# davide-coccomini/MINTIME-Multi-Identity-size-iNvariant-TIMEsformer-for-Video-Deepfake-Detection

Measured on AMD Instinct MI355X. Metric: clips/sec (8-frame, 2-identity, 224^2 crops) fwd+bwd, higher is better.
Workload: dtype f32; 1 GPU; config 3: EfficientNet-B0 + SizeInvariantTimeSformer(dim 512, depth 9, heads 8), B=32/GPU, 8 frames, 2 identities (identity-masked), 224x224 crops, random-init seeded weights (restored before every step), train-mode BN + drop-connect 0.2, step = fwd + BCE loss + bwd + SGD(lr .01, wd 1e-4); global_batch=32, frames=8, parallelism=dp1

## Files before the change

include/mintime_hip.h:

```cpp
#ifndef MINTIME_HIP_H
#define MINTIME_HIP_H
#include <stdint.h>
#ifdef __cplusplus
extern "C" {
#endif

#define MT_VERSION 122

int mt_version(void);
const char* mt_last_error(void);

int mt_set_deterministic(int on);
int mt_get_deterministic(void);
int mt_det_release(void* stream);
int mt_det_bn_sums(const float* x, const float* z, const float* mean_invstd, int64_t rows, int C, int mode, double* stats, void* stream);

typedef struct { int gin, gout, off; } mt_rowmap;

enum { MT_OP_NT = 0,
       MT_OP_NN = 1,
       MT_OP_TN = 2 };

enum { MT_PRO_NONE = 0, MT_PRO_BN_SWISH_GATE = 1, MT_PRO_BN_SWISH = 2, MT_PRO_AFFINE = 3,
       MT_PRO_BN_BWD = 4,
// ... 53 lines not shown
  int epilogue;
  int M, N, K;
  const void* a_planes;
  const void* b_planes;
  float* C; int64_t ldc;
  const float* bias;
  const float* R; int64_t ldr;
  float* C2; int64_t ldc2;
  int n_half;
  float* col_sum;
  void* c_planes;
  int split_k;
  void* sk_workspace;
  int64_t sk_workspace_bytes;
  double* stats; int stats_slots;
} mt_gemm_planes_desc;

int mt_gemm_planes(const mt_gemm_planes_desc* d, void* stream);

int mt_mul_planes(const float* x, const float* m, void* planes, float* out, int rows, int cols, void* stream);
int mt_mul_add(const float* y, const float* m, const float* r, float* out, int64_t n, void* stream);
int mt_geglu_bwd(const float* dh, const float* m, const float* u, void* du_planes, float* du, int rows, int n_half, void* stream);
int64_t mt_gemm_planes_workspace_bytes(void);
int mt_gemm_planes_set_persist(int blocks_per_cu);


int mt_layernorm_fwd(const float* x, const float* gamma, const float* beta, float* y, float* stats,
                     int rows, int dim, float eps, void* y_planes, void* stream);

int mt_embed_fwd(float* x, const float* cls, const float* pos_emb, const float* size_emb,
                 const int64_t* positions, const int32_t* sizes, int B, int F, int n, int dim, int pos_rows, int size_rows,
// ... 232 lines not shown
```

mintime-multi-identity-size-invariant-timesformer-for-video-deepfake-detection_amd/csrc/gemm_planes.hip:

```cpp
#include "../../include/mintime_hip.h"
#include "common.hpp"
#include "gemm_planes_launch.hpp"
#include "gemm_geometry.hpp"
#include "det.hpp"
#include <string.h>

using namespace mt;

namespace {

__device__ __forceinline__ void to_blk_block(const float* __restrict__ src, int64_t ld, int R, int C, const PlaneRef& o, int rb, int cb, int lane) {
  const int r = rb * 32 + (lane >> 1), c = cb * 16 + (lane & 1) * 8;
  float x[8] = {0.f, 0.f, 0.f, 0.f, 0.f, 0.f, 0.f, 0.f};
  if (r < R) {
    const float* s = src + (int64_t)r * ld + c;
    if (c + 8 <= C && ((ld & 3) == 0) && (((uintptr_t)src & 15) == 0)) {
      const float4 u = *reinterpret_cast<const float4*>(s), v = *reinterpret_cast<const float4*>(s + 4);
      x[0] = u.x; x[1] = u.y; x[2] = u.z; x[3] = u.w; x[4] = v.x; x[5] = v.y; x[6] = v.z; x[7] = v.w;
    } else {
#pragma unroll
      for (int e = 0; e < 8; ++e) if (c + e < C) x[e] = s[e];
    }
  }
  planes_store8(o, r, c, x);
// ... 70 lines not shown
}

extern "C" int mt_gemm_planes_set_persist(int blocks_per_cu) {
  const int prev = persist_blocks();
  g_persist = blocks_per_cu < 0 || blocks_per_cu > 4 ? 0 : blocks_per_cu;
  return prev;
}

extern "C" int64_t mt_gemm_planes_workspace_bytes(void) { return kSkFlagBytes + (int64_t)kSkMaxGrid * 128 * 128 * 4; }

extern "C" int64_t mt_planes_elems(int rows, int cols) {
  if (rows <= 0 || cols <= 0) return 0;
  return (int64_t)((rows + 31) & ~31) * ((cols + 15) & ~15);
}

extern "C" int mt_split_planes_blk(const float* src, int64_t ld, int rows, int cols, void* planes, void* stream) {
  if (!src || !planes) return fail(MT_ERR_ARG, "mt_split_planes_blk: null pointer");
  if (rows <= 0 || cols <= 0 || ld < cols) return fail(MT_ERR_ARG, "mt_split_planes_blk: bad shape %d x %d (ld %lld)", rows, cols, (long long)ld);
  if ((uintptr_t)planes & 15) return fail(MT_ERR_ARG, "mt_split_planes_blk: planes must be 16-byte aligned");
  const int cb16 = (cols + 15) >> 4, rp = (rows + 31) & ~31;
  const PlaneRef o{reinterpret_cast<__bf16*>(planes), (int64_t)rp * cb16 * 16, cb16, rp};
  hipLaunchKernelGGL(split_planes_blk_kernel, dim3((cb16 + 3) / 4, rp / 32), dim3(256), 0, (hipStream_t)stream, src, ld, rows, cols, o);
  return check_launch("mt_split_planes_blk");
}

extern "C" int mt_bn_bwd_apply_planes(const float* du, const float* z, const float* kabc, void* planes, int rows, int C, void* stream) {
  if (!du || !z || !kabc || !planes || rows <= 0 || C <= 0) return fail(MT_ERR_ARG, "mt_bn_bwd_apply_planes: bad arguments");
  if ((C & 3) || (((uintptr_t)du | (uintptr_t)z | (uintptr_t)kabc | (uintptr_t)planes) & 15))
    return fail(MT_ERR_ARG, "mt_bn_bwd_apply_planes: C %% 4 == 0 and 16-byte alignment");
  const int cb16 = (C + 15) >> 4, rp = (rows + 31) & ~31;
// ... 4 lines not shown

extern "C" int mt_split_planes_blk_multi(const void* items, int count, int64_t total_blocks, void* stream) {
  if (!items || count <= 0 || total_blocks <= 0) return fail(MT_ERR_ARG, "mt_split_planes_blk_multi: bad arguments");
  hipLaunchKernelGGL(split_planes_blk_multi_kernel, dim3((unsigned)((total_blocks + 3) / 4)), dim3(256), 0, (hipStream_t)stream,
                     reinterpret_cast<const SplitItem*>(items), count, total_blocks);
  return check_launch("mt_split_planes_blk_multi");
}

static int gemm_planes_impl(const mt_gemm_planes_desc* d, void* stream) {
  if (!d || !d->a_planes || !d->b_planes) return fail(MT_ERR_ARG, "mt_gemm_planes: null operand planes");
  if (d->M <= 0 || d->N <= 0 || d->K <= 0) return fail(MT_ERR_ARG, "mt_gemm_planes: bad shape %d %d %d", d->M, d->N, d->K);
  if (((uintptr_t)d->a_planes & 15) || ((uintptr_t)d->b_planes & 15) || ((uintptr_t)d->c_planes & 15))
    return fail(MT_ERR_ARG, "mt_gemm_planes: planes must be 16-byte aligned");
  const int op = d->op, epi = d->epilogue;
  const bool cpl = d->c_planes != nullptr;
  if (!d->C && !cpl) return fail(MT_ERR_ARG, "mt_gemm_planes: no output");
  if (cpl && epi != MT_EPI_GEGLU && epi != MT_EPI_GEGLU_BWD) return fail(MT_ERR_UNSUPPORTED, "mt_gemm_planes: plane output only from the GEGLU pair");
  if (epi == MT_EPI_BIAS_RES && !d->R) return fail(MT_ERR_ARG, "mt_gemm_planes: BIAS_RES needs R");
  if (epi == MT_EPI_GEGLU && (d->n_half * 2 != d->N || (d->n_half & 63))) return fail(MT_ERR_ARG, "mt_gemm_planes GEGLU: N must be 2*n_half, n_half %% 64 == 0");
  if (epi == MT_EPI_GEGLU_BWD && (!d->C2 || d->n_half != d->N || (d->n_half & 31)))
    return fail(MT_ERR_ARG, "mt_gemm_planes GEGLU_BWD: needs C2, n_half == N and n_half %% 32 == 0");
  hipStream_t s = (hipStream_t)stream;
  const bool high = matmul_precision() == MT_PRECISION_HIGH;
  const int np = high ? 2 : 3;
  auto launch = [&](int skm, const GemmArgs& ga, dim3 g) {
    return high ? launch_planes_high(op, epi, cpl, skm, ga, g, s) : launch_planes_form<3>(op, epi, cpl, skm, ga, g, s);
  };

  const int a_rows = op == MT_OP_TN ? d->K : d->M, a_cols = op == MT_OP_TN ? d->M : d->K;
  const int b_rows = op == MT_OP_NT ? d->N : d->K, b_cols = op == MT_OP_NT ? d->K : d->N;
  GemmArgs a;
  memset(&a, 0, sizeof(a));
  a.C = d->C; a.M = d->M; a.N = d->N; a.K = d->K; a.ldc = d->ldc;
  a.a_planes = d->a_planes; a.a_pstride = mt_planes_elems(a_rows, a_cols); a.lda = (a_cols + 15) >> 4;
  a.b_planes = d->b_planes; a.b_pstride = mt_planes_elems(b_rows, b_cols); a.ldb = (b_cols + 15) >> 4;
  if (6 * a.a_pstride > 0xFFFFFFFFll || 6 * a.b_pstride > 0xFFFFFFFFll)
    return fail(MT_ERR_UNSUPPORTED, "mt_gemm_planes: an operand's planes span %lld bytes (> 4 GB: 32-bit DMA offsets); use mt_gemm for it (lib.planes_fit)",
                (long long)(6 * (a.a_pstride > a.b_pstride ? a.a_pstride : a.b_pstride)));
  a.bias = d->bias; a.R = d->R; a.ldr = d->ldr; a.C2 = d->C2; a.ldc2 = d->ldc2; a.n_half = d->n_half; a.col_sum = d->col_sum;
  a.hw = 1; a.stats_slots = d->stats_slots != 0 ? d->stats_slots : 1; a.stats = d->stats; a.b_hw = 1; a.e_hw = 1;
  if (epi == MT_EPI_STATS && !d->stats) return fail(MT_ERR_ARG, "mt_gemm_planes: STATS needs stats");
// ... 53 lines not shown
```

mintime-multi-identity-size-invariant-timesformer-for-video-deepfake-detection_amd/csrc/gemm_planes.hpp:

```cpp
#pragma once
#include "gemm_split.hpp"
#include "planes.hpp"

#ifndef MT_PLANES_ABLATE
#define MT_PLANES_ABLATE 0
#endif
#ifndef MT_PLANES_EPI_ABLATE
#define MT_PLANES_EPI_ABLATE 0
#endif
#ifndef MT_PLANES_PRIO
#define MT_PLANES_PRIO 0
#endif

namespace mt {

typedef short s16x4_t __attribute__((ext_vector_type(4)));
enum : int { BAL_NONE = 0, BAL_PAIR = 1, BAL_PHASE = 2 };

__device__ __forceinline__ void lds_dma16_s(const void* sbase, unsigned voff, unsigned lds_byte_addr) {
  unsigned keep;
  asm volatile("s_mov_b32 %0, m0\n\ts_mov_b32 m0, %3\n\ts_nop 0\n\tglobal_load_lds_dwordx4 %1, %2\n\ts_mov_b32 m0, %0"
               : "=&s"(keep) : "v"(voff), "s"(sbase), "s"(lds_byte_addr) : "memory");
}

// ... 4 lines not shown
  asm volatile("s_waitcnt lgkmcnt(0)" ::: "memory");
#pragma unroll
  for (int pass = 0; pass < 2; ++pass) {
    const int g = pass * 64 + lane, row = g >> 2, cg = g & 3;
    const float4 lo = *reinterpret_cast<const float4*>(wl + row * 36 + cg * 8);
    const float4 hi = *reinterpret_cast<const float4*>(wl + row * 36 + cg * 8 + 4);
    const int rg = row0 + row, cgl = col0 + cg * 8;
    const bool live = rg < M;
    const float x[8] = {live ? lo.x : 0.f, live ? lo.y : 0.f, live ? lo.z : 0.f, live ? lo.w : 0.f,
                        live ? hi.x : 0.f, live ? hi.y : 0.f, live ? hi.z : 0.f, live ? hi.w : 0.f};
    if (rg < o.rows_pad && cgl < o.cb16 * 16) { if (MT_PLANES_EPI_ABLATE & 8) { if (x[0] + x[7] == 123.456f) o.p[0] = (__bf16)1.f; } else planes_store8(o, rg, cgl, x); }
  }
  asm volatile("s_waitcnt lgkmcnt(0)" ::: "memory");
}

template <int TM, int TN, int EPI>
__device__ __forceinline__ void planes_epilogue(const GemmArgs& p, f32x16 (&acc)[TM][TN], int m0, int n0, int wm, int wn, int lane, float* wl) {
  static_assert(EPI == EPI_GEGLU || EPI == EPI_GEGLU_BWD, "plane output: the GEGLU pair");
  const PlaneRef o{reinterpret_cast<__bf16*>(p.c_planes), p.c_pstride, (int)p.ldcp, (p.M + 31) & ~31};
  const int col_l = lane & 31, row_h = (lane >> 5) * 4;
  const int mw = m0 + wm * TM * 32;
  if constexpr (EPI == EPI_GEGLU) {
    const int j = (n0 >> 1) + wn * 32 + col_l;
    const bool jok = j < p.n_half;
    const float ba = (jok && p.bias) ? p.bias[j] : 0.f;
    const float bg = (jok && p.bias) ? p.bias[p.n_half + j] : 0.f;
#pragma unroll
    for (int i = 0; i < TM; ++i) {
      float hv[16];
#pragma unroll
      for (int r = 0; r < 16; ++r) {
        const int m = mw + i * 32 + row_h + (r & 3) + 8 * (r >> 2);
        const float a = acc[i][0][r] + ba, g = acc[i][1][r] + bg;
        hv[r] = a * gelu_erf(g);
        if (m < p.M && jok) {
          if (p.C2) *reinterpret_cast<float2*>(p.C2 + (int64_t)m * p.ldc2 + 2 * j) = make_float2(a, g);
          if (p.C) p.C[(int64_t)m * p.ldc + j] = hv[r];
        }
      }
      planes_emit_tile(hv, wl, o, mw + i * 32, (n0 >> 1) + wn * 32, p.M, lane);
    }
  } else {
    f32x16 dgs[TM][TN];
    float s1[TN], s2[TN];
#pragma unroll
    for (int j = 0; j < TN; ++j) {
      const int n = n0 + wn * TN * 32 + j * 32 + col_l;
      const bool nok = n < p.N;
      s1[j] = 0.f; s2[j] = 0.f;
#pragma unroll
      for (int i = 0; i < TM; ++i) {
        float2 ag[16];
#pragma unroll
        for (int r = 0; r < 16; ++r) {
          const int m = mw + i * 32 + row_h + (r & 3) + 8 * (r >> 2);
          ag[r] = ((MT_PLANES_EPI_ABLATE & 1) || !(m < p.M && nok)) ? make_float2(0.3f, 0.1f)
                                                                     : *reinterpret_cast<const float2*>(p.C2 + (int64_t)m * p.ldc2 + 2 * n);
        }
#pragma unroll
        for (int r = 0; r < 16; ++r) {
          const int m = mw + i * 32 + row_h + (r & 3) + 8 * (r >> 2);
          const float v = acc[i][j][r];
          float gl, gr;
          if (MT_PLANES_EPI_ABLATE & 2) { gl = ag[r].y; gr = ag[r].y + 1.f; } else gelu_erf_both(ag[r].y, gl, gr);
          const bool live = m < p.M && nok;
          const float da = live ? v * gl : 0.f, dg = live ? v * ag[r].x * gr : 0.f;
          acc[i][j][r] = da;
          dgs[i][j][r] = dg;
          s1[j] += da; s2[j] += dg;
        }
        __builtin_amdgcn_sched_barrier(0);
      }
    }
#pragma unroll
    for (int j = 0; j < TN; ++j) {
      const int n = n0 + wn * TN * 32 + j * 32 + col_l;
      const bool nok = n < p.N;
#pragma unroll
      for (int i = 0; i < TM; ++i) {
        float da[16], dg[16];
#pragma unroll
        for (int r = 0; r < 16; ++r) {
          da[r] = acc[i][j][r]; dg[r] = dgs[i][j][r];
          const int m = mw + i * 32 + row_h + (r & 3) + 8 * (r >> 2);
          if (p.C && m < p.M && nok) { p.C[(int64_t)m * p.ldc + n] = da[r]; p.C[(int64_t)m * p.ldc + p.n_half + n] = dg[r]; }
        }
        if (MT_PLANES_EPI_ABLATE & 4) { if (da[3] + dg[5] == 123.456f) p.col_sum[0] = 1.f; }
        else if (n0 + wn * TN * 32 + j * 32 < p.N) {
          planes_emit_tile(da, wl, o, mw + i * 32, n0 + wn * TN * 32 + j * 32, p.M, lane);
          planes_emit_tile(dg, wl, o, mw + i * 32, p.n_half + n0 + wn * TN * 32 + j * 32, p.M, lane);
        }
      }
      if (p.col_sum && !(MT_PLANES_EPI_ABLATE & 16)) {
        float t1 = s1[j], t2 = s2[j];
        t1 += __shfl_xor(t1, 32);
        t2 += __shfl_xor(t2, 32);
        if (lane < 32 && nok) {
          if (p.det.vals) {
            const int rk = mw >> 5;
            det_put(p.det, n >> 5, rk, n & 31, t1);
// ... 25 lines not shown
    const int idx = t - base;
    const int per_group = rows * p.group_n;
    const int g = idx / per_group;
    const int rem = idx - g * per_group;
    const int groups = (n_tiles + p.group_n - 1) / p.group_n;
    const int gw = (g == groups - 1) ? n_tiles - g * p.group_n : p.group_n;
    const int ml = rem / gw;
    mt_ = row0 + ml;
    nt_ = g * p.group_n + (rem - ml * gw);
  } else {
    mt_ = t / n_tiles;
    nt_ = t - mt_ * n_tiles;
  }
}

template <int WAVES_M, int WAVES_N, int TM, int TN, bool AKM, bool BKM, int EPI, int STAGES, int MINW, int BAL, bool CPL = false, int SKM = 0, int NP = 3>
__global__ __launch_bounds__(WAVES_M * WAVES_N * 64, MINW)
void gemm_planes_kernel(const GemmArgs p) {
  constexpr int NW = WAVES_M * WAVES_N;
  constexpr int BM = WAVES_M * TM * 32;
  constexpr int BN = WAVES_N * TN * 32;
  constexpr int BK = 16;
  constexpr int A_PLANE = BM * 32, B_PLANE = BN * 32;
  static_assert(NP == 2 || NP == 3, "two or three pieces per operand");
  constexpr int STAGE = NP * (A_PLANE + B_PLANE);
  constexpr int PPA = A_PLANE / 1024, PPB = B_PLANE / 1024;
  constexpr int PA = NP * PPA, PB = NP * PPB;
  static_assert((PA + PB) % NW == 0, "every wavefront must issue the same number of DMA pieces");
  constexpr int IPW = (PA + PB) / NW;
  static_assert(STAGES >= 2 && STAGES <= 4, "2..4 stages");
  static_assert((!AKM || BM == 128) && (!BKM || BN == 128), "k-major images are laid out for 128-column tiles");
  constexpr bool SK = SKM == 1, PS = SKM == 2;
  static_assert(!SK || !AKM, "stream-K: forward / data-gradient forms (weight gradients split K over the grid already)");
  static_assert(!PS || (!AKM && !CPL && STAGES == 2 && EPI != EPI_GEGLU && BAL != BAL_PHASE), "persistent form: NT / NN, fp32 output, ring of two");
  constexpr bool PAIR = BAL == BAL_PAIR, PHASE = BAL == BAL_PHASE;

  extern __shared__ __attribute__((aligned(16))) unsigned char smem_pl[];
  const unsigned lds_base = (unsigned)(uintptr_t)(__attribute__((address_space(3))) unsigned char*)smem_pl;

// ... 246 lines not shown
      float sacc = 0.f;
#pragma unroll
      for (int i = 0; i < TM; ++i)
#pragma unroll
        for (int j = 0; j < TN; ++j)
#pragma unroll
          for (int r = 0; r < 16; ++r) sacc += acc[i][j][r];
      if (sacc == 123.456f) p.C[0] = sacc;
      return;
    }
    int m0e = mt_ * BM, n0e = nt_ * BN, lane_e = lane;
    asm volatile("" : "+s"(m0e), "+s"(n0e), "+v"(lane_e));
    if constexpr (CPL) {
      static_assert(!CPL || STAGES * STAGE >= NW * 32 * 36 * 4, "the plane epilogue's LDS patches live in the main loop's stages");
      __syncthreads();
      planes_epilogue<TM, TN, EPI>(p, acc, m0e, n0e, wm, wn, lane_e, reinterpret_cast<float*>(smem_pl) + wave * (32 * 36));
    } else {
      gemm_epilogue<TM, TN, EPI>(p, acc, m0e, n0e, wm, wn, lane_e, split_idx);
    }
  };

  if (p.wave_prio == 1) __builtin_amdgcn_s_setprio(1);
  else if (p.wave_prio == 2) __builtin_amdgcn_s_setprio(2);
  else if (p.wave_prio == 3) __builtin_amdgcn_s_setprio(3);
  if (MT_PLANES_PRIO == 1) {
    const unsigned hwid = __builtin_amdgcn_s_getreg((4 << 0) | (0 << 6) | (3 << 11));
    if (__builtin_amdgcn_readfirstlane(hwid) & 1) __builtin_amdgcn_s_setprio(1);
  } else if (MT_PLANES_PRIO == 2) {
    if ((blockIdx.x >> 8) & 1) __builtin_amdgcn_s_setprio(1);
  }

// ... 220 lines not shown
```

mintime-multi-identity-size-invariant-timesformer-for-video-deepfake-detection_amd/csrc/gemm_planes_high.hip:

```cpp
#include "gemm_planes_launch.hpp"

namespace mt {

int launch_planes_high(int op, int epi, bool cpl, int skm, const GemmArgs& a, dim3 grid, hipStream_t s) {
  return launch_planes_form<2>(op, epi, cpl, skm, a, grid, s);
}

}
```

mintime-multi-identity-size-invariant-timesformer-for-video-deepfake-detection_amd/csrc/gemm_planes_launch.hpp:

```cpp
#pragma once
#include "../../include/mintime_hip.h"
#include "common.hpp"
#include "gemm_planes.hpp"

#ifndef MT_PLANES_HIGH_STAGES
#define MT_PLANES_HIGH_STAGES 3
#endif

namespace mt {

template <int NP, bool AKM, bool BKM, int EPI, int BAL, bool CPL, int SK = 0>
int launch_planes(const GemmArgs& a, dim3 grid, hipStream_t s) {
  constexpr int ST = (NP == 2 && SK != 2) ? MT_PLANES_HIGH_STAGES : 2;
  auto k = gemm_planes_kernel<2, 2, 2, 2, AKM, BKM, EPI, ST, BAL == BAL_PAIR ? 2 : 3, BAL, CPL, SK, NP>;
  constexpr size_t lds = (size_t)ST * NP * (128 + 128) * 32;
  {
    hipError_t e = ensure_dynamic_lds(reinterpret_cast<const void*>(k), lds);
    if (e != hipSuccess) return fail(MT_ERR_LAUNCH, "mt_gemm_planes: cannot reserve %zu B of LDS: %s", lds, hipGetErrorString(e));
  }
  hipLaunchKernelGGL(k, grid, dim3(256), lds, s, a);
  return check_launch("mt_gemm_planes");
}

template <int NP>
int launch_planes_form(int op, int epi, bool cpl, int skm, const GemmArgs& a, dim3 grid, hipStream_t s) {
  if (op == MT_OP_TN && epi == MT_EPI_ATOMIC) return launch_planes<NP, true, true, EPI_ATOMIC, BAL_NONE, false, 0>(a, grid, s);
  if (skm == 2 && !cpl) {
    if (op == MT_OP_NT && epi == MT_EPI_STORE) return launch_planes<NP, false, false, EPI_STORE, BAL_PAIR, false, 2>(a, grid, s);
    if (op == MT_OP_NT && epi == MT_EPI_BIAS_RES) return launch_planes<NP, false, false, EPI_BIAS_RES, BAL_PAIR, false, 2>(a, grid, s);
    if (op == MT_OP_NN && epi == MT_EPI_STORE) return launch_planes<NP, false, true, EPI_STORE, BAL_PAIR, false, 2>(a, grid, s);
  }
  if (skm == 0 || skm == 1) {
#define PL_COMBO(OP, BKM_, EPI_, CPL_)                                                               \
  if (op == OP && epi == EPI_ && cpl == CPL_)                                                        \
    return skm ? launch_planes<NP, false, BKM_, EPI_, BAL_PAIR, CPL_, 1>(a, grid, s)                 \
               : launch_planes<NP, false, BKM_, EPI_, BAL_PAIR, CPL_, 0>(a, grid, s);
    PL_COMBO(MT_OP_NT, false, EPI_STORE, false)
    PL_COMBO(MT_OP_NT, false, EPI_BIAS_RES, false)
    PL_COMBO(MT_OP_NT, false, EPI_STATS, false)
    PL_COMBO(MT_OP_NT, false, EPI_GEGLU, false)
    PL_COMBO(MT_OP_NT, false, EPI_GEGLU, true)
    PL_COMBO(MT_OP_NN, true, EPI_STORE, false)
    PL_COMBO(MT_OP_NN, true, EPI_BIAS_RES, false)
    PL_COMBO(MT_OP_NN, true, EPI_GEGLU_BWD, false)
    PL_COMBO(MT_OP_NN, true, EPI_GEGLU_BWD, true)
#undef PL_COMBO
  }
  return fail(MT_ERR_UNSUPPORTED, "mt_gemm_planes: unsupported op / epilogue %d / %d", op, epi);
}

int launch_planes_high(int op, int epi, bool cpl, int skm, const GemmArgs& a, dim3 grid, hipStream_t s);

}
```

mintime-multi-identity-size-invariant-timesformer-for-video-deepfake-detection_amd/lib.py:

```python
import ctypes as C
import os
import subprocess
import threading

import torch

_HERE = os.path.dirname(os.path.abspath(__file__))
CSRC = os.path.join(_HERE, "csrc")
LIB_PATH = os.environ.get("MT_LIB") or os.path.join(CSRC, "libmintime_hip.so")

_lib = None

f32p = C.c_void_p
i64 = C.c_int64


class RowMap(C.Structure):
    _fields_ = [("gin", C.c_int), ("gout", C.c_int), ("off", C.c_int)]


class Conv3dDesc(C.Structure):
    _fields_ = [(n, C.c_int) for n in ("N", "T", "H", "W", "C", "To", "Ho", "Wo", "K", "kt", "kh", "kw", "st", "sh", "sw", "pt", "ph",
                                       "pw")] + [("ldx", i64), ("ldy", i64)]

# ... 10 lines not shown
                ("n_half", C.c_int), ("split_k", C.c_int),
                ("A2", C.c_void_p), ("b_prologue", C.c_int), ("b_scale", C.c_void_p), ("b_shift", C.c_void_p),
                ("b_gate", C.c_void_p), ("b_hw", C.c_int),
                ("conv_H", C.c_int), ("conv_W", C.c_int), ("conv_C", C.c_int), ("conv_Ho", C.c_int), ("conv_Wo", C.c_int),
                ("conv_k", C.c_int), ("conv_stride", C.c_int), ("conv_pad", C.c_int), ("conv_act", C.c_int), ("conv_src_u8", C.c_int),
                ("col_sum", C.c_void_p), ("b_planes", C.c_void_p), ("b_plane_stride", C.c_int64),
                ("e_scale", C.c_void_p), ("e_shift", C.c_void_p), ("e_gate", C.c_void_p), ("e_dpool", C.c_void_p),
                ("e_mi", C.c_void_p), ("e_hw", C.c_int)]


class GemmPlanesDesc(C.Structure):
    _fields_ = [("op", C.c_int), ("epilogue", C.c_int), ("M", C.c_int), ("N", C.c_int), ("K", C.c_int),
                ("a_planes", C.c_void_p), ("b_planes", C.c_void_p), ("C", C.c_void_p), ("ldc", i64),
                ("bias", C.c_void_p), ("R", C.c_void_p), ("ldr", i64), ("C2", C.c_void_p), ("ldc2", i64),
                ("n_half", C.c_int), ("col_sum", C.c_void_p), ("c_planes", C.c_void_p), ("split_k", C.c_int),
                ("sk_workspace", C.c_void_p), ("sk_workspace_bytes", i64), ("stats", C.c_void_p), ("stats_slots", C.c_int)]


OP_NT, OP_NN, OP_TN = 0, 1, 2
PRO_NONE, PRO_BN_SWISH_GATE, PRO_BN_SWISH, PRO_AFFINE, PRO_BN_BWD, PRO_IM2COL = 0, 1, 2, 3, 4, 5
BPRO_NONE, BPRO_BN_SWISH_GATE, BPRO_IM2COL = 0, 1, 2
EPI_STORE, EPI_BIAS_RES, EPI_GEGLU, EPI_STATS, EPI_ATOMIC, EPI_GEGLU_BWD, EPI_ACCUM, EPI_SE_RED, EPI_ACT_BWD = 0, 1, 2, 3, 4, 5, 6, 7, 8

PROTOTYPES = {
    "mt_version": [],
    "mt_last_error": [],
    "mt_set_deterministic": [C.c_int],
    "mt_get_deterministic": [],
    "mt_det_release": [C.c_void_p],
    "mt_det_bn_sums": [f32p, f32p, f32p, i64, C.c_int, C.c_int, C.c_void_p, C.c_void_p],
    "mt_gemm": [C.POINTER(GemmDesc), C.c_void_p],
    "mt_gemm_set_split": [C.c_int],
    "mt_gemm_get_split": [],
    "mt_gemm_set_precision": [C.c_int],
    "mt_gemm_get_precision": [],
    "mt_split_planes": [f32p, C.c_void_p, C.c_int64, C.c_void_p],
    "mt_planes_elems": [C.c_int, C.c_int],
    "mt_split_planes_blk": [f32p, i64, C.c_int, C.c_int, C.c_void_p, C.c_void_p],
    "mt_split_planes_blk_multi": [C.c_void_p, C.c_int, i64, C.c_void_p],
    "mt_bn_bwd_apply_planes": [f32p, f32p, f32p, C.c_void_p, C.c_int, C.c_int, C.c_void_p],
    "mt_gemm_planes": [C.POINTER(GemmPlanesDesc), C.c_void_p],
    "mt_gemm_planes_workspace_bytes": [],
    "mt_gemm_planes_set_persist": [C.c_int],
    "mt_mul_planes": [f32p, f32p, C.c_void_p, f32p, C.c_int, C.c_int, C.c_void_p],
    "mt_mul_add": [f32p, f32p, f32p, f32p, i64, C.c_void_p],
    "mt_geglu_bwd": [f32p, f32p, f32p, C.c_void_p, f32p, C.c_int, C.c_int, C.c_void_p],
    "mt_layernorm_fwd": [f32p, f32p, f32p, f32p, f32p, C.c_int, C.c_int, C.c_float, C.c_void_p, C.c_void_p],
    "mt_embed_fwd": [f32p, f32p, f32p, f32p, C.c_void_p, C.c_void_p, C.c_int, C.c_int, C.c_int, C.c_int, C.c_int, C.c_int, C.c_void_p,
                     C.c_void_p],
    "mt_attn_fwd": [f32p, f32p, f32p, C.c_void_p, C.c_void_p, C.c_int, C.c_int, C.c_int, C.c_int, C.c_int, C.c_float,
                    C.c_void_p, C.c_void_p],
    "mt_head_fwd": [f32p, f32p, f32p, f32p, f32p, f32p, C.c_int, C.c_int, C.c_int, C.c_int, C.c_float, C.c_void_p],
# ... 95 lines not shown
    "mt_sf_ingest_resize_bwd": [f32p, f32p, C.c_void_p, C.c_void_p] + [C.c_int] * 6 + [C.c_void_p, C.c_void_p, f32p] * 2 + [C.c_int] * 7 +
                               [f32p, i64, i64, i64, i64, i64, C.c_void_p],
    "mt_sf_stem_dgrad": [f32p, i64, f32p, f32p] + [C.c_int] * 6 + [C.c_void_p],
    "mt_plan_create": [C.POINTER(C.c_void_p)],
    "mt_plan_destroy": [C.c_void_p],
    "mt_plan_record_begin": [C.c_void_p],
    "mt_plan_record_end": [C.c_void_p],
    "mt_plan_size": [C.c_void_p],
    "mt_plan_tag": [C.c_int, C.c_double],
    "mt_plan_fork": [C.c_void_p, C.c_void_p],
    "mt_plan_run": [C.c_void_p, C.c_uint],
    "mt_plan_probe_read": [C.c_void_p, C.c_int, C.POINTER(C.c_int), C.POINTER(C.c_double), C.POINTER(C.c_double)],
    "mt_memset_async": [C.c_void_p, C.c_int, i64, C.c_void_p],
    "mt_copy_async": [C.c_void_p, C.c_void_p, i64, C.c_void_p],
}
_RESTYPES = {"mt_last_error": C.c_char_p, "mt_planes_elems": C.c_int64, "mt_gemm_planes_workspace_bytes": C.c_int64,
             "mt_conv3d_part_floats": C.c_int64, "mt_sf_bn_bwd_part_floats": C.c_int64}


class MintimeHipError(RuntimeError):
    pass


def build(verbose: bool = False):
    cmd = ["make", "-C", CSRC, "-j", str(min(16, os.cpu_count() or 4))]
    res = subprocess.run(cmd, capture_output=True, text=True)
    if res.returncode != 0:
        raise MintimeHipError("building libmintime_hip.so failed:\n" + res.stdout[-4000:] + res.stderr[-8000:])
    if verbose:
        print(res.stdout[-2000:])
    global _lib
# ... 125 lines not shown
    if ws is None:
        if torch.cuda.is_current_stream_capturing():
            return None
        n = get().mt_gemm_planes_workspace_bytes()
        ws = torch.zeros(n, dtype=torch.uint8, device=st.device)
        _SK_WORKSPACES[key] = ws
    return ws


def planes_fit(rows: int, cols: int) -> bool:
    rp, cp = (rows + 31) // 32 * 32, (cols + 15) // 16 * 16
    return 6 * rp * cp <= 0xFFFFFFFF


def gemm_planes(op, a_planes, b_planes, M, N, K, Cout=None, ldc=0, epilogue=EPI_STORE, bias=None, R=None, ldr=0, C2=None, ldc2=0,
                n_half=0, col_sum=None, c_planes=None, split_k=0, streamk=None, stats=None, stats_slots=0):
    d = GemmPlanesDesc()
    if streamk is None:
        streamk = os.environ.get("MT_PLANES_STREAMK", "0") != "0"
    if streamk and op != OP_TN:
        ws = streamk_workspace(a_planes.device)
        if ws is not None:
            d.sk_workspace, d.sk_workspace_bytes = ptr(ws), ws.numel()
    d.op, d.epilogue, d.M, d.N, d.K = op, epilogue, M, N, K
    d.a_planes, d.b_planes, d.C, d.ldc = ptr(a_planes), ptr(b_planes), ptr(Cout), ldc
    d.bias, d.R, d.ldr, d.C2, d.ldc2 = ptr(bias), ptr(R), ldr, ptr(C2), ldc2
    d.n_half, d.col_sum, d.c_planes, d.split_k = n_half, ptr(col_sum), ptr(c_planes), split_k
    d.stats, d.stats_slots = ptr(stats), stats_slots
    if recording() is not None:
        if op == OP_TN:
            tag_next(TAG_WGRAD, 2.0 * M * N * K)
        elif epilogue == EPI_GEGLU:
            tag_next(TAG_FF1, 2.0 * M * N * K)
    prof = PROFILE
    if prof is not None:
        for pr in prof:
            if "match_planes" in pr and pr["match_planes"](d):
                e0, e1 = torch.cuda.Event(enable_timing=True), torch.cuda.Event(enable_timing=True)
                e0.record()
                check(get().mt_gemm_planes(C.byref(d), stream_ptr()), "mt_gemm_planes")
                e1.record()
                pr["events"].append((e0, e1, 2.0 * M * N * K))
                return
# ... 282 lines not shown
```

mintime-multi-identity-size-invariant-timesformer-for-video-deepfake-detection_amd/tsf_planes.py:

```python
import os

import torch

from . import arch
from . import lib as L
from . import plans
from .lib import _new

_SEL = (2, 3, 7, 8, 12, 14)


def eligible(model, M, save):
    if os.environ.get("MT_TSF_PLANES", "1") == "0" or not L.gemm_split_enabled():
        return False
    if os.environ.get("MT_TSF_PRUNE_LAST", "0") != "0":
        return False
    if torch.cuda.is_current_stream_capturing() and save:
        return False
    D, inner = model.dim, model.heads * model.dim_head
    return (M >= 512 or dropout_active(model)) and D % 16 == 0 and inner % 16 == 0 and model.dim_head == 64


def dropout_active(model):
    return model.training and (float(model.attn_dropout) > 0.0 or float(model.ff_dropout) > 0.0)
# ... 87 lines not shown
            dm = None
            if p_att > 0.0:
                dm = _dropout_mult(model, (M, D), p_att, dev)
                y0 = _new(dev, M, D)
                L.gemm_planes(L.OP_NT, o_p, wp[(li, 3 if mode == 0 else 8)], M, D, inner, Cout=y0, ldc=D, bias=b_o)
                L.check(lib.mt_mul_add(L.ptr(y0), L.ptr(dm), L.ptr(x), L.ptr(x_new), M * D, st), "mt_mul_add")
            else:
                L.gemm_planes(L.OP_NT, o_p, wp[(li, 3 if mode == 0 else 8)], M, D, inner, Cout=x_new, ldc=D, epilogue=L.EPI_BIAS_RES,
                              bias=b_o, R=x, ldr=D)
            if save:
                rec[mode] = dict(x=x, stats=stats, xn_p=xn_p, qkv=qkv, o_p=o_p, dm=dm)
            x = x_new
        g, b_, w1, b1, w2, b2 = next(it), next(it), next(it), next(it), next(it), next(it)
        if save:
            xn_p, h_p, stats = L.planes_empty(M, D, dev), L.planes_empty(M, 4 * D, dev), _new(dev, M, 2)
            u = _new(dev, M, 8 * D)
        else:
            stats, u = None, None
        L.check(lib.mt_layernorm_fwd(L.ptr(x), L.ptr(g), L.ptr(b_), None, L.ptr(stats), M, D, eps, L.ptr(xn_p), st), "mt_layernorm_fwd")
        dm = None
        if p_ff > 0.0:
            dm = _dropout_mult(model, (M, 4 * D), p_ff, dev)
            h = _new(dev, M, 4 * D)
            L.gemm_planes(L.OP_NT, xn_p, wp[(li, 12)], M, 8 * D, D, epilogue=L.EPI_GEGLU, bias=b1, C2=u, ldc2=8 * D, n_half=4 * D,
                          Cout=h, ldc=4 * D)
            L.check(lib.mt_mul_planes(L.ptr(h), L.ptr(dm), L.ptr(h_p), None, M, 4 * D, st), "mt_mul_planes")
            del h
        else:
            L.gemm_planes(L.OP_NT, xn_p, wp[(li, 12)], M, 8 * D, D, epilogue=L.EPI_GEGLU, bias=b1, C2=u, ldc2=8 * D, n_half=4 * D,
                          c_planes=h_p)
        x_new = _new(dev, B, N, D) if save else x
        L.gemm_planes(L.OP_NT, h_p, wp[(li, 14)], M, D, 4 * D, Cout=x_new, ldc=D, epilogue=L.EPI_BIAS_RES, bias=b2, R=x, ldr=D)
        if save:
            rec[2] = dict(x=x, stats=stats, xn_p=xn_p, u=u, h_p=h_p, dm=dm)
            saved["layers"].append(rec)
        x = x_new
    g, b_, w_h, b_h = next(it), next(it), next(it), next(it)
    logits = _new(dev, B, model.num_classes)
    L.check(lib.mt_head_fwd(L.ptr(x), L.ptr(g), L.ptr(b_), L.ptr(w_h), L.ptr(b_h), L.ptr(logits), B, x.shape[1], D, model.num_classes,
                            eps, st), "mt_head_fwd")
    if save:
        saved["x_final"] = x
    return logits, s_att, t_att, saved


# ... 63 lines not shown
        i0 = take(6)
        g, b_, w1, b1, w2, b2 = P[i0:i0 + 6]
        r = rec[2]
        du_p = L.planes_empty(M, 8 * D, dev)
        dxn = torch.empty(M, D, dtype=torch.float32, device=dev)
        last = li == model.depth - 1
        wgrad(dx_p, r["h_p"], grads[i0 + 4], D, 4 * D, bias_src=dx2 if last else None, bias_out=grads[i0 + 5] if last else None)
        if r.get("dm") is not None:
            dh, du_f = torch.empty(M, 4 * D, dtype=torch.float32, device=dev), torch.empty(M, 8 * D, dtype=torch.float32, device=dev)
            L.gemm_planes(L.OP_NN, dx_p, wp[(li, 14)], M, 4 * D, D, Cout=dh, ldc=4 * D)
            L.check(lib.mt_geglu_bwd(L.ptr(dh), L.ptr(r["dm"]), L.ptr(r["u"]), L.ptr(du_p), L.ptr(du_f), M, 4 * D, st), "mt_geglu_bwd")
            side.launch(lambda du_f=du_f, out=grads[i0 + 3]: L.check(lib.mt_colsum(L.ptr(du_f), 8 * D, L.RowMap(0, 0, 0), M, 8 * D,
                                                                                 L.ptr(out), L.stream_ptr()), "mt_colsum"), reads=(du_f,))
            del dh
        else:
            L.gemm_planes(L.OP_NN, dx_p, wp[(li, 14)], M, 4 * D, D, epilogue=L.EPI_GEGLU_BWD, C2=r["u"], ldc2=8 * D, n_half=4 * D,
                          col_sum=grads[i0 + 3], c_planes=du_p)
        wgrad(du_p, r["xn_p"], grads[i0 + 2], 8 * D, D)
        L.gemm_planes(L.OP_NN, du_p, wp[(li, 12)], M, D, 8 * D, Cout=dxn, ldc=D)
        dx2, dx_p = ln_bwd(dxn, r, g, dx2, i0, None if rec[1].get("dm") is not None else grads[i0 - 1], 0)
        if not keep_saved:
            r.clear()
        for mode in (1, 0):
            i0 = take(5)
            g, b_, w_qkv, w_o, b_o = P[i0:i0 + 5]
            r = rec[mode]
            dxn = torch.empty(M, D, dtype=torch.float32, device=dev)
            dy_p = dx_p
            if r.get("dm") is not None:
                dy_p = L.planes_empty(M, D, dev)
                dy_f = torch.empty(M, D, dtype=torch.float32, device=dev)
                L.check(lib.mt_mul_planes(L.ptr(dx2), L.ptr(r["dm"]), L.ptr(dy_p), L.ptr(dy_f), M, D, st), "mt_mul_planes")
# ... 41 lines not shown
```

Baseline: 726.3 clips/s.

## Store GEGLU pre-activations in MFMA-tile order for coalesced fwd/bwd epilogue access

The GEGLU forward epilogue now writes the saved pre-activations (a, g) in a 32x32 tile-blocked layout that matches the MFMA accumulator lane order, using float4 stores. The GEGLU backward epilogue reads them back with float4 loads instead of strided per-row float2 gathers. This targets the scattered memory traffic of the large M x 8D saved tensor in both passes. It adds a C2T template variant, a new workspace-size helper and API field, and a tiled buffer that is used only when feed-forward dropout is off.

```diff
diff --git a/include/mintime_hip.h b/include/mintime_hip.h
--- a/include/mintime_hip.h
+++ b/include/mintime_hip.h
@@ -91,7 +91,10 @@
   void* sk_workspace;
   int64_t sk_workspace_bytes;
   double* stats; int stats_slots;
+  int c2_tiled;
 } mt_gemm_planes_desc;
+
+int64_t mt_geglu_tiled_elems(int M, int n_half);
 
 int mt_gemm_planes(const mt_gemm_planes_desc* d, void* stream);
 
diff --git a/mintime-multi-identity-size-invariant-timesformer-for-video-deepfake-detection_amd/csrc/gemm_planes.hip b/mintime-multi-identity-size-invariant-timesformer-for-video-deepfake-detection_amd/csrc/gemm_planes.hip
--- a/mintime-multi-identity-size-invariant-timesformer-for-video-deepfake-detection_amd/csrc/gemm_planes.hip
+++ b/mintime-multi-identity-size-invariant-timesformer-for-video-deepfake-detection_amd/csrc/gemm_planes.hip
@@ -108,6 +108,11 @@
   return (int64_t)((rows + 31) & ~31) * ((cols + 15) & ~15);
 }
 
+extern "C" int64_t mt_geglu_tiled_elems(int M, int n_half) {
+  if (M <= 0 || n_half <= 0 || (n_half & 31)) return 0;
+  return (int64_t)((M + 31) & ~31) * 2 * n_half;
+}
+
 extern "C" int mt_split_planes_blk(const float* src, int64_t ld, int rows, int cols, void* planes, void* stream) {
   if (!src || !planes) return fail(MT_ERR_ARG, "mt_split_planes_blk: null pointer");
   if (rows <= 0 || cols <= 0 || ld < cols) return fail(MT_ERR_ARG, "mt_split_planes_blk: bad shape %d x %d (ld %lld)", rows, cols, (long long)ld);
@@ -142,6 +147,10 @@
     return fail(MT_ERR_ARG, "mt_gemm_planes: planes must be 16-byte aligned");
   const int op = d->op, epi = d->epilogue;
   const bool cpl = d->c_planes != nullptr;
+  const bool c2t = d->c2_tiled != 0;
+  if (c2t && (d->c2_tiled != 1 || !((op == MT_OP_NT && epi == MT_EPI_GEGLU) || (op == MT_OP_NN && epi == MT_EPI_GEGLU_BWD)) || !cpl || !d->C2 ||
+              ((uintptr_t)d->C2 & 15)))
+    return fail(MT_ERR_ARG, "mt_gemm_planes: c2_tiled = 1 needs the GEGLU (NT) / GEGLU_BWD (NN) epilogue, c_planes and a 16-byte aligned C2");
   if (!d->C && !cpl) return fail(MT_ERR_ARG, "mt_gemm_planes: no output");
   if (cpl && epi != MT_EPI_GEGLU && epi != MT_EPI_GEGLU_BWD) return fail(MT_ERR_UNSUPPORTED, "mt_gemm_planes: plane output only from the GEGLU pair");
   if (epi == MT_EPI_BIAS_RES && !d->R) return fail(MT_ERR_ARG, "mt_gemm_planes: BIAS_RES needs R");
@@ -152,7 +161,7 @@
   const bool high = matmul_precision() == MT_PRECISION_HIGH;
   const int np = high ? 2 : 3;
   auto launch = [&](int skm, const GemmArgs& ga, dim3 g) {
-    return high ? launch_planes_high(op, epi, cpl, skm, ga, g, s) : launch_planes_form<3>(op, epi, cpl, skm, ga, g, s);
+    return high ? launch_planes_high(op, epi, cpl, skm, c2t, ga, g, s) : launch_planes_form<3>(op, epi, cpl, skm, c2t, ga, g, s);
   };
 
   const int a_rows = op == MT_OP_TN ? d->K : d->M, a_cols = op == MT_OP_TN ? d->M : d->K;
diff --git a/mintime-multi-identity-size-invariant-timesformer-for-video-deepfake-detection_amd/csrc/gemm_planes.hpp b/mintime-multi-identity-size-invariant-timesformer-for-video-deepfake-detection_amd/csrc/gemm_planes.hpp
--- a/mintime-multi-identity-size-invariant-timesformer-for-video-deepfake-detection_amd/csrc/gemm_planes.hpp
+++ b/mintime-multi-identity-size-invariant-timesformer-for-video-deepfake-detection_amd/csrc/gemm_planes.hpp
@@ -42,7 +42,7 @@
   asm volatile("s_waitcnt lgkmcnt(0)" ::: "memory");
 }
 
-template <int TM, int TN, int EPI>
+template <int TM, int TN, int EPI, bool C2T>
 __device__ __forceinline__ void planes_epilogue(const GemmArgs& p, f32x16 (&acc)[TM][TN], int m0, int n0, int wm, int wn, int lane, float* wl) {
   static_assert(EPI == EPI_GEGLU || EPI == EPI_GEGLU_BWD, "plane output: the GEGLU pair");
   const PlaneRef o{reinterpret_cast<__bf16*>(p.c_planes), p.c_pstride, (int)p.ldcp, (p.M + 31) & ~31};
@@ -56,14 +56,27 @@
 #pragma unroll
     for (int i = 0; i < TM; ++i) {
       float hv[16];
+      [[maybe_unused]] float ua[16], ug[16];
 #pragma unroll
       for (int r = 0; r < 16; ++r) {
         const int m = mw + i * 32 + row_h + (r & 3) + 8 * (r >> 2);
         const float a = acc[i][0][r] + ba, g = acc[i][1][r] + bg;
         hv[r] = a * gelu_erf(g);
+        if constexpr (C2T) { ua[r] = m < p.M ? a : 0.f; ug[r] = m < p.M ? g : 0.f; }
         if (m < p.M && jok) {
-          if (p.C2) *reinterpret_cast<float2*>(p.C2 + (int64_t)m * p.ldc2 + 2 * j) = make_float2(a, g);
+          if constexpr (!C2T) { if (p.C2) *reinterpret_cast<float2*>(p.C2 + (int64_t)m * p.ldc2 + 2 * j) = make_float2(a, g); }
           if (p.C) p.C[(int64_t)m * p.ldc + j] = hv[r];
+        }
+      }
+      if constexpr (C2T) {
+        const int rb = (mw + i * 32) >> 5, jb = ((n0 >> 1) + wn * 32) >> 5;
+        if (rb * 32 < p.M && jb * 32 < p.n_half) {
+          float* ub = p.C2 + ((int64_t)rb * (p.n_half >> 5) + jb) * 2048 + lane * 4;
+#pragma unroll
+          for (int q = 0; q < 4; ++q) {
+            *reinterpret_cast<float4*>(ub + q * 256) = make_float4(ua[4 * q], ua[4 * q + 1], ua[4 * q + 2], ua[4 * q + 3]);
+            *reinterpret_cast<float4*>(ub + 1024 + q * 256) = make_float4(ug[4 * q], ug[4 * q + 1], ug[4 * q + 2], ug[4 * q + 3]);
+          }
         }
       }
       planes_emit_tile(hv, wl, o, mw + i * 32, (n0 >> 1) + wn * 32, p.M, lane);
@@ -79,11 +92,23 @@
 #pragma unroll
       for (int i = 0; i < TM; ++i) {
         float2 ag[16];
-#pragma unroll
-        for (int r = 0; r < 16; ++r) {
-          const int m = mw + i * 32 + row_h + (r & 3) + 8 * (r >> 2);
-          ag[r] = ((MT_PLANES_EPI_ABLATE & 1) || !(m < p.M && nok)) ? make_float2(0.3f, 0.1f)
-                                                                     : *reinterpret_cast<const float2*>(p.C2 + (int64_t)m * p.ldc2 + 2 * n);
+        if constexpr (C2T) {
+          const int rb = min((mw + i * 32) >> 5, ((p.M + 31) >> 5) - 1), jb = min((n0 + wn * TN * 32 + j * 32) >> 5, (p.n_half >> 5) - 1);
+          const float* ub = p.C2 + ((int64_t)rb * (p.n_half >> 5) + jb) * 2048 + lane * 4;
+#pragma unroll
+          for (int q = 0; q < 4; ++q) {
+            float4 a4 = make_float4(0.3f, 0.3f, 0.3f, 0.3f), g4 = make_float4(0.1f, 0.1f, 0.1f, 0.1f);
+            if (!(MT_PLANES_EPI_ABLATE & 1)) { a4 = *reinterpret_cast<const float4*>(ub + q * 256); g4 = *reinterpret_cast<const float4*>(ub + 1024 + q * 256); }
+            ag[4 * q] = make_float2(a4.x, g4.x); ag[4 * q + 1] = make_float2(a4.y, g4.y);
+            ag[4 * q + 2] = make_float2(a4.z, g4.z); ag[4 * q + 3] = make_float2(a4.w, g4.w);
+          }
+        } else {
+#pragma unroll
+          for (int r = 0; r < 16; ++r) {
+            const int m = mw + i * 32 + row_h + (r & 3) + 8 * (r >> 2);
+            ag[r] = ((MT_PLANES_EPI_ABLATE & 1) || !(m < p.M && nok)) ? make_float2(0.3f, 0.1f)
+                                                                       : *reinterpret_cast<const float2*>(p.C2 + (int64_t)m * p.ldc2 + 2 * n);
+          }
         }
 #pragma unroll
         for (int r = 0; r < 16; ++r) {
@@ -100,6 +125,7 @@
         __builtin_amdgcn_sched_barrier(0);
       }
     }
+    asm volatile("" ::: "memory");
 #pragma unroll
     for (int j = 0; j < TN; ++j) {
       const int n = n0 + wn * TN * 32 + j * 32 + col_l;
@@ -110,8 +136,14 @@
 #pragma unroll
         for (int r = 0; r < 16; ++r) {
           da[r] = acc[i][j][r]; dg[r] = dgs[i][j][r];
-          const int m = mw + i * 32 + row_h + (r & 3) + 8 * (r >> 2);
-          if (p.C && m < p.M && nok) { p.C[(int64_t)m * p.ldc + n] = da[r]; p.C[(int64_t)m * p.ldc + p.n_half + n] = dg[r]; }
+        }
+        if (p.C) {
+          float* cp = p.C + (int64_t)(mw + i * 32 + row_h) * p.ldc + n;
+#pragma unroll
+          for (int r = 0; r < 16; ++r) {
+            const int dr = (r & 3) + 8 * (r >> 2);
+            if (mw + i * 32 + row_h + dr < p.M && nok) { cp[(int64_t)dr * p.ldc] = da[r]; cp[(int64_t)dr * p.ldc + p.n_half] = dg[r]; }
+          }
         }
         if (MT_PLANES_EPI_ABLATE & 4) { if (da[3] + dg[5] == 123.456f) p.col_sum[0] = 1.f; }
         else if (n0 + wn * TN * 32 + j * 32 < p.N) {
@@ -167,7 +199,7 @@
   }
 }
 
-template <int WAVES_M, int WAVES_N, int TM, int TN, bool AKM, bool BKM, int EPI, int STAGES, int MINW, int BAL, bool CPL = false, int SKM = 0, int NP = 3>
+template <int WAVES_M, int WAVES_N, int TM, int TN, bool AKM, bool BKM, int EPI, int STAGES, int MINW, int BAL, bool CPL = false, int SKM = 0, int NP = 3, bool C2T = false>
 __global__ __launch_bounds__(WAVES_M * WAVES_N * 64, MINW)
 void gemm_planes_kernel(const GemmArgs p) {
   constexpr int NW = WAVES_M * WAVES_N;
@@ -176,6 +208,7 @@
   constexpr int BK = 16;
   constexpr int A_PLANE = BM * 32, B_PLANE = BN * 32;
   static_assert(NP == 2 || NP == 3, "two or three pieces per operand");
+  static_assert(!C2T || (CPL && (EPI == EPI_GEGLU || EPI == EPI_GEGLU_BWD)), "tiled pre-activations: the plane epilogues of the GEGLU pair");
   constexpr int STAGE = NP * (A_PLANE + B_PLANE);
   constexpr int PPA = A_PLANE / 1024, PPB = B_PLANE / 1024;
   constexpr int PA = NP * PPA, PB = NP * PPB;
@@ -452,7 +485,7 @@
     if constexpr (CPL) {
       static_assert(!CPL || STAGES * STAGE >= NW * 32 * 36 * 4, "the plane epilogue's LDS patches live in the main loop's stages");
       __syncthreads();
-      planes_epilogue<TM, TN, EPI>(p, acc, m0e, n0e, wm, wn, lane_e, reinterpret_cast<float*>(smem_pl) + wave * (32 * 36));
+      planes_epilogue<TM, TN, EPI, C2T>(p, acc, m0e, n0e, wm, wn, lane_e, reinterpret_cast<float*>(smem_pl) + wave * (32 * 36));
     } else {
       gemm_epilogue<TM, TN, EPI>(p, acc, m0e, n0e, wm, wn, lane_e, split_idx);
     }
diff --git a/mintime-multi-identity-size-invariant-timesformer-for-video-deepfake-detection_amd/csrc/gemm_planes_high.hip b/mintime-multi-identity-size-invariant-timesformer-for-video-deepfake-detection_amd/csrc/gemm_planes_high.hip
--- a/mintime-multi-identity-size-invariant-timesformer-for-video-deepfake-detection_amd/csrc/gemm_planes_high.hip
+++ b/mintime-multi-identity-size-invariant-timesformer-for-video-deepfake-detection_amd/csrc/gemm_planes_high.hip
@@ -2,8 +2,8 @@
 
 namespace mt {
 
-int launch_planes_high(int op, int epi, bool cpl, int skm, const GemmArgs& a, dim3 grid, hipStream_t s) {
-  return launch_planes_form<2>(op, epi, cpl, skm, a, grid, s);
+int launch_planes_high(int op, int epi, bool cpl, int skm, bool c2t, const GemmArgs& a, dim3 grid, hipStream_t s) {
+  return launch_planes_form<2>(op, epi, cpl, skm, c2t, a, grid, s);
 }
 
 }
diff --git a/mintime-multi-identity-size-invariant-timesformer-for-video-deepfake-detection_amd/csrc/gemm_planes_launch.hpp b/mintime-multi-identity-size-invariant-timesformer-for-video-deepfake-detection_amd/csrc/gemm_planes_launch.hpp
--- a/mintime-multi-identity-size-invariant-timesformer-for-video-deepfake-detection_amd/csrc/gemm_planes_launch.hpp
+++ b/mintime-multi-identity-size-invariant-timesformer-for-video-deepfake-detection_amd/csrc/gemm_planes_launch.hpp
@@ -9,10 +9,10 @@
 
 namespace mt {
 
-template <int NP, bool AKM, bool BKM, int EPI, int BAL, bool CPL, int SK = 0>
+template <int NP, bool AKM, bool BKM, int EPI, int BAL, bool CPL, int SK = 0, bool C2T = false>
 int launch_planes(const GemmArgs& a, dim3 grid, hipStream_t s) {
   constexpr int ST = (NP == 2 && SK != 2) ? MT_PLANES_HIGH_STAGES : 2;
-  auto k = gemm_planes_kernel<2, 2, 2, 2, AKM, BKM, EPI, ST, BAL == BAL_PAIR ? 2 : 3, BAL, CPL, SK, NP>;
+  auto k = gemm_planes_kernel<2, 2, 2, 2, AKM, BKM, EPI, ST, BAL == BAL_PAIR ? 2 : 3, BAL, CPL, SK, NP, C2T>;
   constexpr size_t lds = (size_t)ST * NP * (128 + 128) * 32;
   {
     hipError_t e = ensure_dynamic_lds(reinterpret_cast<const void*>(k), lds);
@@ -23,7 +23,19 @@
 }
 
 template <int NP>
-int launch_planes_form(int op, int epi, bool cpl, int skm, const GemmArgs& a, dim3 grid, hipStream_t s) {
+int launch_planes_form(int op, int epi, bool cpl, int skm, bool c2t, const GemmArgs& a, dim3 grid, hipStream_t s) {
+  if (c2t) {
+    if (cpl && (skm == 0 || skm == 1)) {
+#define PL_TILED(OP, BKM_, EPI_)                                                                     \
+  if (op == OP && epi == EPI_)                                                                       \
+    return skm ? launch_planes<NP, false, BKM_, EPI_, BAL_PAIR, true, 1, true>(a, grid, s)           \
+               : launch_planes<NP, false, BKM_, EPI_, BAL_PAIR, true, 0, true>(a, grid, s);
+      PL_TILED(MT_OP_NT, false, EPI_GEGLU)
+      PL_TILED(MT_OP_NN, true, EPI_GEGLU_BWD)
+#undef PL_TILED
+    }
+    return fail(MT_ERR_UNSUPPORTED, "mt_gemm_planes: tiled pre-activations with op / epilogue %d / %d", op, epi);
+  }
   if (op == MT_OP_TN && epi == MT_EPI_ATOMIC) return launch_planes<NP, true, true, EPI_ATOMIC, BAL_NONE, false, 0>(a, grid, s);
   if (skm == 2 && !cpl) {
     if (op == MT_OP_NT && epi == MT_EPI_STORE) return launch_planes<NP, false, false, EPI_STORE, BAL_PAIR, false, 2>(a, grid, s);
@@ -49,6 +61,6 @@
   return fail(MT_ERR_UNSUPPORTED, "mt_gemm_planes: unsupported op / epilogue %d / %d", op, epi);
 }
 
-int launch_planes_high(int op, int epi, bool cpl, int skm, const GemmArgs& a, dim3 grid, hipStream_t s);
+int launch_planes_high(int op, int epi, bool cpl, int skm, bool c2t, const GemmArgs& a, dim3 grid, hipStream_t s);
 
 }
diff --git a/mintime-multi-identity-size-invariant-timesformer-for-video-deepfake-detection_amd/lib.py b/mintime-multi-identity-size-invariant-timesformer-for-video-deepfake-detection_amd/lib.py
--- a/mintime-multi-identity-size-invariant-timesformer-for-video-deepfake-detection_amd/lib.py
+++ b/mintime-multi-identity-size-invariant-timesformer-for-video-deepfake-detection_amd/lib.py
@@ -48,7 +48,8 @@
                 ("a_planes", C.c_void_p), ("b_planes", C.c_void_p), ("C", C.c_void_p), ("ldc", i64),
                 ("bias", C.c_void_p), ("R", C.c_void_p), ("ldr", i64), ("C2", C.c_void_p), ("ldc2", i64),
                 ("n_half", C.c_int), ("col_sum", C.c_void_p), ("c_planes", C.c_void_p), ("split_k", C.c_int),
-                ("sk_workspace", C.c_void_p), ("sk_workspace_bytes", i64), ("stats", C.c_void_p), ("stats_slots", C.c_int)]
+                ("sk_workspace", C.c_void_p), ("sk_workspace_bytes", i64), ("stats", C.c_void_p), ("stats_slots", C.c_int),
+                ("c2_tiled", C.c_int)]
 
 
 OP_NT, OP_NN, OP_TN = 0, 1, 2
@@ -70,6 +71,7 @@
     "mt_gemm_get_precision": [],
     "mt_split_planes": [f32p, C.c_void_p, C.c_int64, C.c_void_p],
     "mt_planes_elems": [C.c_int, C.c_int],
+    "mt_geglu_tiled_elems": [C.c_int, C.c_int],
     "mt_split_planes_blk": [f32p, i64, C.c_int, C.c_int, C.c_void_p, C.c_void_p],
     "mt_split_planes_blk_multi": [C.c_void_p, C.c_int, i64, C.c_void_p],
     "mt_bn_bwd_apply_planes": [f32p, f32p, f32p, C.c_void_p, C.c_int, C.c_int, C.c_void_p],
@@ -195,7 +197,7 @@
     "mt_memset_async": [C.c_void_p, C.c_int, i64, C.c_void_p],
     "mt_copy_async": [C.c_void_p, C.c_void_p, i64, C.c_void_p],
 }
-_RESTYPES = {"mt_last_error": C.c_char_p, "mt_planes_elems": C.c_int64, "mt_gemm_planes_workspace_bytes": C.c_int64,
+_RESTYPES = {"mt_last_error": C.c_char_p, "mt_planes_elems": C.c_int64, "mt_geglu_tiled_elems": C.c_int64, "mt_gemm_planes_workspace_bytes": C.c_int64,
              "mt_conv3d_part_floats": C.c_int64, "mt_sf_bn_bwd_part_floats": C.c_int64}
 
 
@@ -351,7 +353,7 @@
 
 
 def gemm_planes(op, a_planes, b_planes, M, N, K, Cout=None, ldc=0, epilogue=EPI_STORE, bias=None, R=None, ldr=0, C2=None, ldc2=0,
-                n_half=0, col_sum=None, c_planes=None, split_k=0, streamk=None, stats=None, stats_slots=0):
+                n_half=0, col_sum=None, c_planes=None, split_k=0, streamk=None, stats=None, stats_slots=0, c2_tiled=0):
     d = GemmPlanesDesc()
     if streamk is None:
         streamk = os.environ.get("MT_PLANES_STREAMK", "0") != "0"
@@ -363,7 +365,7 @@
     d.a_planes, d.b_planes, d.C, d.ldc = ptr(a_planes), ptr(b_planes), ptr(Cout), ldc
     d.bias, d.R, d.ldr, d.C2, d.ldc2 = ptr(bias), ptr(R), ldr, ptr(C2), ldc2
     d.n_half, d.col_sum, d.c_planes, d.split_k = n_half, ptr(col_sum), ptr(c_planes), split_k
-    d.stats, d.stats_slots = ptr(stats), stats_slots
+    d.stats, d.stats_slots, d.c2_tiled = ptr(stats), stats_slots, c2_tiled
     if recording() is not None:
         if op == OP_TN:
             tag_next(TAG_WGRAD, 2.0 * M * N * K)
diff --git a/mintime-multi-identity-size-invariant-timesformer-for-video-deepfake-detection_amd/tsf_planes.py b/mintime-multi-identity-size-invariant-timesformer-for-video-deepfake-detection_amd/tsf_planes.py
--- a/mintime-multi-identity-size-invariant-timesformer-for-video-deepfake-detection_amd/tsf_planes.py
+++ b/mintime-multi-identity-size-invariant-timesformer-for-video-deepfake-detection_amd/tsf_planes.py
@@ -125,7 +125,7 @@
         g, b_, w1, b1, w2, b2 = next(it), next(it), next(it), next(it), next(it), next(it)
         if save:
             xn_p, h_p, stats = L.planes_empty(M, D, dev), L.planes_empty(M, 4 * D, dev), _new(dev, M, 2)
-            u = _new(dev, M, 8 * D)
+            u = _new(dev, M, 8 * D) if p_ff > 0.0 else _new(dev, lib.mt_geglu_tiled_elems(M, 4 * D))
         else:
             stats, u = None, None
         L.check(lib.mt_layernorm_fwd(L.ptr(x), L.ptr(g), L.ptr(b_), None, L.ptr(stats), M, D, eps, L.ptr(xn_p), st), "mt_layernorm_fwd")
@@ -138,8 +138,8 @@
             L.check(lib.mt_mul_planes(L.ptr(h), L.ptr(dm), L.ptr(h_p), None, M, 4 * D, st), "mt_mul_planes")
             del h
         else:
-            L.gemm_planes(L.OP_NT, xn_p, wp[(li, 12)], M, 8 * D, D, epilogue=L.EPI_GEGLU, bias=b1, C2=u, ldc2=8 * D, n_half=4 * D,
-                          c_planes=h_p)
+            L.gemm_planes(L.OP_NT, xn_p, wp[(li, 12)], M, 8 * D, D, epilogue=L.EPI_GEGLU, bias=b1, C2=u, n_half=4 * D,
+                          c_planes=h_p, c2_tiled=int(u is not None))
         x_new = _new(dev, B, N, D) if save else x
         L.gemm_planes(L.OP_NT, h_p, wp[(li, 14)], M, D, 4 * D, Cout=x_new, ldc=D, epilogue=L.EPI_BIAS_RES, bias=b2, R=x, ldr=D)
         if save:
@@ -233,8 +233,8 @@
                                                                                  L.ptr(out), L.stream_ptr()), "mt_colsum"), reads=(du_f,))
             del dh
         else:
-            L.gemm_planes(L.OP_NN, dx_p, wp[(li, 14)], M, 4 * D, D, epilogue=L.EPI_GEGLU_BWD, C2=r["u"], ldc2=8 * D, n_half=4 * D,
-                          col_sum=grads[i0 + 3], c_planes=du_p)
+            L.gemm_planes(L.OP_NN, dx_p, wp[(li, 14)], M, 4 * D, D, epilogue=L.EPI_GEGLU_BWD, C2=r["u"], n_half=4 * D,
+                          col_sum=grads[i0 + 3], c_planes=du_p, c2_tiled=1)
         wgrad(du_p, r["xn_p"], grads[i0 + 2], 8 * D, D)
         L.gemm_planes(L.OP_NN, du_p, wp[(li, 12)], M, D, 8 * D, Cout=dxn, ldc=D)
         dx2, dx_p = ln_bwd(dxn, r, g, dx2, i0, None if rec[1].get("dm") is not None else grads[i0 - 1], 0)
```

After: 732.6 clips/s, median of 6. No clear change (+0.9%).
